# gau-nernst/pytorch-models

Hardware: AMD Instinct MI355X
Metric: ViT-B/16 images/s & Whisper-base audio-sec/s (BASELINE.json metric; value / unit / ms_per_step = the ViT-B/16 leg of configs[1], the Whisper-base leg of configs[2] is the "whisper" object) (higher is better)
Workload: dtype bf16; 1 GPU; ViT-B/16 bf16 forward, batch=256 per GPU, 224x224 (BASELINE configs[1]); per_gpu_batch=256, global_batch=256, parallelism=dp1, collective=none

## Files before the change

pytorch-models_amd/csrc/common.h:

```cpp
#pragma once
#include <hip/hip_runtime.h>
#include <stdint.h>

#include "../../include/pm_mi355x.h"

typedef __bf16 bf16;
typedef __attribute__((ext_vector_type(8))) __bf16 bf16x8;
typedef __attribute__((ext_vector_type(4))) __bf16 bf16x4;
typedef __attribute__((ext_vector_type(2))) __bf16 bf16x2;
typedef __attribute__((ext_vector_type(4))) float f32x4;
typedef __attribute__((ext_vector_type(2))) float f32x2;
typedef __attribute__((ext_vector_type(16))) float f32x16;
typedef __attribute__((ext_vector_type(4))) short s16x4;

#define PM_LDS __attribute__((address_space(3)))
#define PM_GLOBAL __attribute__((address_space(1)))

__device__ __forceinline__ float sum8_dpp(float v) {
  v += __builtin_bit_cast(float, __builtin_amdgcn_update_dpp(0, __builtin_bit_cast(int, v), 0xB1, 0xF, 0xF, true));
  v += __builtin_bit_cast(float, __builtin_amdgcn_update_dpp(0, __builtin_bit_cast(int, v), 0x4E, 0xF, 0xF, true));
  v += __builtin_bit_cast(float, __builtin_amdgcn_update_dpp(0, __builtin_bit_cast(int, v), 0x141, 0xF, 0xF, true));
  return v;
}

struct PmLnFold {
  const float* stats;
  const float* s;
  float* row_out;
};

#define PM_CHECK_LAUNCH()                                  \
  do {                                                     \
    if (hipGetLastError() != hipSuccess) return PM_ELAUNCH; \
  } while (0)

__device__ __forceinline__ float bf16_bits_to_f32(unsigned short b) { return __uint_as_float(((unsigned)b) << 16); }

#ifndef PM_GLDS_AUX
#define PM_GLDS_AUX 0
#endif
#ifndef PM_Y_NT
#define PM_Y_NT 1
#endif
template <typename V>
__device__ __forceinline__ void store_y(V* p, V v) {
#if PM_Y_NT
  __builtin_nontemporal_store(v, p);
#else
  *p = v;
#endif
}
__device__ __forceinline__ void glds16(const void* gsrc, void* lds_dst_wave_base) {
  __builtin_amdgcn_global_load_lds((const PM_GLOBAL void*)gsrc, (PM_LDS void*)lds_dst_wave_base, 16, 0, PM_GLDS_AUX);
}
#ifndef PM_GLDS_X_AUX
#define PM_GLDS_X_AUX 0
#endif
#ifndef PM_GLDS_W_AUX
#define PM_GLDS_W_AUX 0
#endif
template <int AUX>
__device__ __forceinline__ void glds16_aux(const void* gsrc, void* lds_dst_wave_base) {
  __builtin_amdgcn_global_load_lds((const PM_GLOBAL void*)gsrc, (PM_LDS void*)lds_dst_wave_base, 16, 0, AUX);
}

__device__ __forceinline__ void store_sc1_x4(f32x4* p, f32x4 v) {
  asm volatile("global_store_dwordx4 %0, %1, off sc1" ::"v"(p), "v"(v) : "memory");
}
__device__ __forceinline__ f32x4 load_sc1_x4(const f32x4* p) {
  f32x4 v;
  asm volatile("global_load_dwordx4 %0, %1, off sc1\n\ts_waitcnt vmcnt(0)" : "=v"(v) : "v"(p) : "memory");
  return v;
}

__device__ __forceinline__ f32x4 load_sc1_x4_async(const f32x4* p) {
  f32x4 v;
  asm volatile("global_load_dwordx4 %0, %1, off sc1" : "=v"(v) : "v"(p) : "memory");
  return v;
}
__device__ __forceinline__ void wait_loads(f32x4& a, f32x4& b, f32x4& c, f32x4& d) {
  asm volatile("s_waitcnt vmcnt(0)" : "+v"(a), "+v"(b), "+v"(c), "+v"(d)::"memory");
}

__device__ __forceinline__ void wait_vmcnt0() { asm volatile("s_waitcnt vmcnt(0)" ::: "memory"); }

__device__ __forceinline__ float erf_fast(float x) {
  const float ax = fabsf(x);
  const float t = __frcp_rn(fmaf(0.3275911f, ax, 1.0f));
  float p = fmaf(1.061405429f, t, -1.453152027f);
  p = fmaf(p, t, 1.421413741f);
  p = fmaf(p, t, -0.284496736f);
  p = fmaf(p, t, 0.254829592f);
  const float e = __expf(-ax * ax);
  const float r = fmaf(-p * t, e, 1.0f);
  return copysignf(r, x);
}

__device__ __forceinline__ float gelu_poly(float x) {
  const float xc = __builtin_amdgcn_fmed3f(x, -4.5f, 4.5f);
  const float t = fmaf(xc * xc, 2.0f / 20.25f, -1.0f);
  float q = 3.353692146e-03f;
  q = fmaf(q, t, -9.328538250e-03f);
  q = fmaf(q, t, 1.220852128e-02f);
  q = fmaf(q, t, -1.674404426e-02f);
  q = fmaf(q, t, 2.762940359e-02f);
  q = fmaf(q, t, -4.055576763e-02f);
  q = fmaf(q, t, 5.481856801e-02f);
  q = fmaf(q, t, -7.717196008e-02f);
  q = fmaf(q, t, 1.569021127e-01f);
  return x * fmaf(xc, q, 0.5f);
}

__device__ __forceinline__ f32x2 gelu_poly2(f32x2 x) {
  f32x2 xc;
  xc[0] = __builtin_amdgcn_fmed3f(x[0], -4.5f, 4.5f);
  xc[1] = __builtin_amdgcn_fmed3f(x[1], -4.5f, 4.5f);
  const f32x2 k1 = {2.0f / 20.25f, 2.0f / 20.25f}, m1 = {-1.0f, -1.0f}, half = {0.5f, 0.5f};
  const f32x2 t = __builtin_elementwise_fma(xc * xc, k1, m1);
  f32x2 q = {3.353692146e-03f, 3.353692146e-03f};
  q = __builtin_elementwise_fma(q, t, f32x2{-9.328538250e-03f, -9.328538250e-03f});
  q = __builtin_elementwise_fma(q, t, f32x2{1.220852128e-02f, 1.220852128e-02f});
  q = __builtin_elementwise_fma(q, t, f32x2{-1.674404426e-02f, -1.674404426e-02f});
  q = __builtin_elementwise_fma(q, t, f32x2{2.762940359e-02f, 2.762940359e-02f});
  q = __builtin_elementwise_fma(q, t, f32x2{-4.055576763e-02f, -4.055576763e-02f});
  q = __builtin_elementwise_fma(q, t, f32x2{5.481856801e-02f, 5.481856801e-02f});
  q = __builtin_elementwise_fma(q, t, f32x2{-7.717196008e-02f, -7.717196008e-02f});
  q = __builtin_elementwise_fma(q, t, f32x2{1.569021127e-01f, 1.569021127e-01f});
  return x * __builtin_elementwise_fma(xc, q, half);
// ... 53 lines not shown
```

pytorch-models_amd/csrc/linear_bf16.hip:

```cpp
#include <stdlib.h>

#include "common.h"
#ifndef PM_STATIC_PRIO
#define PM_STATIC_PRIO 1
#endif

int pm_linear_bf16_wide_launch(const void* x, int64_t ldx, int64_t x_rows_per_batch, int64_t x_batch_stride, const void* w,
                               int64_t ldw, const float* bias, const void* resid, int64_t ldr, int64_t resid_period, void* y,
                               int64_t ldy, int64_t M, int64_t N, int64_t K, int act, PmLnFold ln, hipStream_t st);
bool pm_linear_bf16_wide_applies(int64_t M, int64_t N, int64_t K, int act);
int pm_linear_bf16_tile_launch(int mi, const void* x, int64_t ldx, int64_t x_rows_per_batch, int64_t x_batch_stride,
                               const void* w, int64_t ldw, const float* bias, const void* resid, int64_t ldr,
                               int64_t resid_period, void* y, int64_t ldy, int64_t M, int64_t N, int64_t K, int act, PmLnFold ln,
                               hipStream_t st);
bool pm_linear_bf16_tile_applies(int64_t M, int64_t N, int64_t K, int act);
#ifdef PM_EXPERIMENTS
int pm_linear_bf16_sk_launch(const void* x, int64_t ldx, int64_t x_rows_per_batch, int64_t x_batch_stride, const void* w,
                             int64_t ldw, const float* bias, const void* resid, int64_t ldr, int64_t resid_period, void* y,
                             int64_t ldy, int64_t M, int64_t N, int64_t K, int act, PmLnFold ln, void* ws, hipStream_t st,
                             int mode);
bool pm_linear_bf16_hyb_applies(int64_t M, int64_t N, int64_t K, int act);
bool pm_linear_bf16_sk_applies(int64_t M, int64_t N, int64_t K, int act);
int64_t pm_linear_sk_ws_bytes();
#else
// ... 427 lines not shown
#undef PM_GO
  return PM_OK;
}

}

enum { PM_K_SMALL = 1, PM_K_PERSIST = 2, PM_K_WIDE = 3, PM_K_SK = 4, PM_K_HYB = 5, PM_K_TILE4 = 6, PM_K_TILE5 = 7 };
static int pm_linear_pick_kernel(int64_t M, int64_t N, int64_t K, bool persist_ok, bool wide_ok, bool sk_ok, bool hyb_ok,
                                 bool has_resid, bool tile_ok) {
  static const int forced = [] { const char* e = getenv("PM_GEMM_KERNEL"); return e ? atoi(e) : 0; }();
  static const bool use_sk = [] { const char* e = getenv("PM_GEMM_STREAMK"); return e && atoi(e) != 0; }();
  if (!use_sk && forced != PM_K_SK) sk_ok = false;
  static const bool use_hyb = [] { const char* e = getenv("PM_GEMM_HYBRID"); return e && atoi(e) != 0; }();
  if (!use_hyb && forced != PM_K_HYB) hyb_ok = false;
  if (forced == PM_K_SK && sk_ok) return PM_K_SK;
  if (forced == PM_K_HYB && hyb_ok) return PM_K_HYB;
  if (forced && forced != PM_K_SK) sk_ok = false;
  if (forced && forced != PM_K_HYB) hyb_ok = false;
  if (forced == PM_K_WIDE && wide_ok) return PM_K_WIDE;
  if ((forced == PM_K_TILE4 || forced == PM_K_TILE5) && tile_ok) return forced;
  static const bool use_tile = [] { const char* e = getenv("PM_GEMM_TILE"); return !e || atoi(e) != 0; }();
  if (!use_tile || forced) tile_ok = false;
  if (forced == PM_K_PERSIST && persist_ok) return PM_K_PERSIST;
  if (forced == PM_K_SMALL) return PM_K_SMALL;
  if (forced == PM_K_PERSIST) wide_ok = false;
  const double tm = (double)((M + 255) / 256), tw = tm * (double)((N + 255) / 256), tp = tm * (double)((N + 127) / 128);
  const double ts = (double)((M + 127) / 128) * (double)((N + 127) / 128);
  auto rounds = [](double t, double slots, double frac) {
    const double full = (double)(int64_t)(t / slots), rem = t - full * slots;
    return full + (rem > 0 ? frac + (1.0 - frac) * rem / slots : 0.0);
  };
  const double cs = rounds(ts, 512, 0.3) * 2.0 / (has_resid ? 0.65 : 0.7);
  const double cp = persist_ok ? rounds(tp, 256, 1.0) * 2.0 : 1e30;
  const double cw = wide_ok ? rounds(tw, 256, 1.0) * 4.0 / (has_resid ? 1.1 : 1.25) : 1e30;
  const double csk = sk_ok ? (tw / 256.0 + 0.25 * 768.0 / (double)K) * 4.0 / (has_resid ? 1.1 : 1.25) : 1e30;
  const double t5 = (double)((M + 319) / 320) * (double)((N + 255) / 256);
  const double ct4 = tile_ok ? rounds(tw, 256, 1.0) * 4.0 / (has_resid ? 1.1 : 1.25) : 1e30;
  const double ct5 = tile_ok ? rounds(t5, 256, 1.0) * 5.0 / (1.07 * (has_resid ? 1.1 : 1.25)) : 1e30;
  if (tile_ok) {
    const double bt = ct4 <= ct5 ? ct4 : ct5;
    if (bt <= cp && bt <= cs) return ct4 <= ct5 ? PM_K_TILE4 : PM_K_TILE5;
  }
  const double best = cw < cp ? (cw < cs ? cw : cs) : (cp < cs ? cp : cs);
  const double chyb = hyb_ok ? ((double)(int64_t)(tw / 256.0) + 0.5 + 0.25 * 768.0 / (double)K) * 4.0 / (has_resid ? 1.1 : 1.25) : 1e30;
  if (csk < 0.97 * best && csk <= chyb) return PM_K_SK;
  if (chyb < 0.97 * best) return PM_K_HYB;
  if (cw <= cp && cw <= cs) return PM_K_WIDE;
  return cp <= cs ? PM_K_PERSIST : PM_K_SMALL;
}

static int linear_impl(const void* x, int64_t ldx, int64_t x_rows_per_batch, int64_t x_batch_stride, const void* w,
                       int64_t ldw, const float* bias, const void* resid, int64_t ldr, int resid_dtype,
                       int64_t resid_period, void* y, int64_t ldy, int y_dtype, int64_t M, int64_t N, int64_t K, int act,
                       PmLnFold ln, void* stream, void* ws = nullptr, int64_t ws_bytes = 0) {
  if (!x || !w || !y || M < 0 || N <= 0 || K <= 0) return PM_EINVAL;
  const bool want_ln = ln.stats || ln.row_out;
  if ((ln.stats == nullptr) != (ln.s == nullptr)) return PM_EINVAL;
  if (ln.row_out && N % 64) return PM_EUNSUPPORTED;
  if (M == 0) return PM_OK;
  if (y_dtype != PM_BF16 && y_dtype != PM_F32) return PM_EINVAL;
  if (resid && resid_dtype != PM_BF16 && resid_dtype != PM_F32) return PM_EINVAL;
  if (K % 8 != 0) return PM_EUNSUPPORTED;
  if (ldx < 0 || ldw < K || ldy < N || (resid && ldr < N) || x_rows_per_batch < 0 || resid_period < 0) return PM_EINVAL;
  if (ldx % 8 || ldw % 8 || x_batch_stride % 8) return PM_EALIGN;
  if (((uintptr_t)x | (uintptr_t)w) & 15) return PM_EALIGN;
  const int vec_ok = (N % 4 == 0) && (ldy % 4 == 0) && (!resid || ldr % 4 == 0) &&
                     !((uintptr_t)y & (y_dtype == PM_F32 ? 15 : 7)) && !(bias && ((uintptr_t)bias & 15)) &&
                     !(resid && ((uintptr_t)resid & (resid_dtype == PM_F32 ? 15 : 7)));
  if (M > (1 << 30) || N > (1 << 30) || K > (1 << 30) || resid_period > (1 << 30)) return PM_EINVAL;
  hipStream_t st0 = (hipStream_t)stream;
  const bool out_vec16 = N % 8 == 0 && ldy % 8 == 0 && !((uintptr_t)y & 15);
  const bool wide_base = y_dtype == PM_BF16 && vec_ok && out_vec16 && !(resid && resid_dtype != PM_BF16) &&
                         !(resid && (ldr % 8 || ((uintptr_t)resid & 15))) &&
                         (x_rows_per_batch > 0 ? (M / x_rows_per_batch + 1) * x_batch_stride : M * ldx) < (1LL << 32) &&
                         N * ldw < (1LL << 32);
  bool wide_ok = wide_base && pm_linear_bf16_wide_applies(M, N, K, act) && !ln.row_out;
  const bool sk_ok = wide_base && ws && ws_bytes >= pm_linear_sk_ws_bytes() && !((uintptr_t)ws & 15) &&
                     pm_linear_bf16_sk_applies(M, N, K, act) && !(ln.row_out && act != PM_ACT_NONE);
  const bool persist_ok = (K % BK == 0) && (M >= 4096) && (y_dtype == PM_F32 || !vec_ok || out_vec16);
  const bool staged_ok = persist_ok && y_dtype == PM_BF16 && vec_ok && !(resid && resid_dtype == PM_F32);
  const bool hyb_ok = wide_base && ws && ws_bytes >= pm_linear_sk_ws_bytes() && !((uintptr_t)ws & 15) &&
                      pm_linear_bf16_hyb_applies(M, N, K, act) && !(ln.row_out && act != PM_ACT_NONE);
  const bool tile_ok = wide_base && pm_linear_bf16_tile_applies(M, N, K, act) && M % 8 == 0 && x_rows_per_batch == 0 &&
                       !(ln.stats && (resid || ln.row_out)) && !(ln.row_out && act != PM_ACT_NONE);
  int kernel;
  if (want_ln) {
    if (!staged_ok) return PM_EUNSUPPORTED;
    kernel = pm_linear_pick_kernel(M, N, K, true, wide_ok, sk_ok, hyb_ok, resid != nullptr, tile_ok);
    if (kernel == PM_K_SMALL) kernel = PM_K_PERSIST;
  } else {
    kernel = pm_linear_pick_kernel(M, N, K, persist_ok, wide_ok, sk_ok, hyb_ok, resid != nullptr, tile_ok);
  }
  if (kernel == PM_K_TILE4 || kernel == PM_K_TILE5) {
    const int rct = pm_linear_bf16_tile_launch(kernel == PM_K_TILE4 ? 4 : 5, x, ldx, x_rows_per_batch, x_batch_stride, w, ldw, bias,
                                               resid, ldr, resid_period, y, ldy, M, N, K, act, ln, st0);
    if (rct != PM_OK) return rct;
    PM_CHECK_LAUNCH();
    return PM_OK;
  }
  if (kernel == PM_K_SK || kernel == PM_K_HYB) {
    const int rck = pm_linear_bf16_sk_launch(x, ldx, x_rows_per_batch, x_batch_stride, w, ldw, bias, resid, ldr, resid_period, y,
                                             ldy, M, N, K, act, ln, ws, st0, kernel == PM_K_HYB ? 1 : 0);
    if (rck != PM_OK) return rck;
    PM_CHECK_LAUNCH();
    return PM_OK;
  }
  if (kernel == PM_K_WIDE) {
    const int rcw = pm_linear_bf16_wide_launch(x, ldx, x_rows_per_batch, x_batch_stride, w, ldw, bias, resid, ldr, resid_period, y,
                                               ldy, M, N, K, act, ln, st0);
    if (rcw != PM_OK) return rcw;
    PM_CHECK_LAUNCH();
    return PM_OK;
  }
  const bool big = kernel == PM_K_PERSIST;
  const int tiles_m = (int)((M + (big ? LBM : BM) - 1) / (big ? LBM : BM)), tiles_n = (int)((N + BN - 1) / BN);
  const int64_t nblk = (int64_t)tiles_m * tiles_n;
  if (nblk > 0x7fffffff) return PM_EINVAL;
  dim3 grid((unsigned)nblk);
  hipStream_t st = (hipStream_t)stream;
  int rc = (y_dtype == PM_F32)
               ? launch_act<true>(act, big, grid, st, (const bf16*)x, ldx, (const bf16*)w, ldw, bias, resid, ldr,
                                  resid_dtype == PM_F32, (int)resid_period, y, ldy, (int)M, (int)N, (int)K, tiles_n,
                                  (int)x_rows_per_batch, x_batch_stride, vec_ok, ln)
               : launch_act<false>(act, big, grid, st, (const bf16*)x, ldx, (const bf16*)w, ldw, bias, resid, ldr,
                                   resid_dtype == PM_F32, (int)resid_period, y, ldy, (int)M, (int)N, (int)K, tiles_n,
                                   (int)x_rows_per_batch, x_batch_stride, vec_ok, ln);
  if (rc != PM_OK) return rc;
  PM_CHECK_LAUNCH();
  return PM_OK;
}

extern "C" int pm_linear_bf16(const void* x, int64_t ldx, const void* w, int64_t ldw, const float* bias,
                              const void* resid, int64_t ldr, int resid_dtype, void* y, int64_t ldy, int y_dtype,
                              int64_t M, int64_t N, int64_t K, int act, void* stream) {
  if (ldx < K) return PM_EINVAL;
  return linear_impl(x, ldx, 0, 0, w, ldw, bias, resid, ldr, resid_dtype, 0, y, ldy, y_dtype, M, N, K, act, PmLnFold{}, stream);
}

extern "C" int pm_linear_bf16_ex(const void* x, int64_t ldx, int64_t x_rows_per_batch, int64_t x_batch_stride,
                                 const void* w, int64_t ldw, const float* bias, const void* resid, int64_t ldr,
                                 int resid_dtype, int64_t resid_period, void* y, int64_t ldy, int y_dtype, int64_t M,
                                 int64_t N, int64_t K, int act, void* stream) {
  return linear_impl(x, ldx, x_rows_per_batch, x_batch_stride, w, ldw, bias, resid, ldr, resid_dtype, resid_period, y, ldy,
                     y_dtype, M, N, K, act, PmLnFold{}, stream);
}

extern "C" int pm_linear_bf16_ln(const void* x, int64_t ldx, int64_t x_rows_per_batch, int64_t x_batch_stride,
                                 const void* w, int64_t ldw, const float* bias, const void* resid, int64_t ldr,
                                 int resid_dtype, int64_t resid_period, void* y, int64_t ldy, int y_dtype, int64_t M,
                                 int64_t N, int64_t K, int act, const float* ln_stats, const float* ln_s,
                                 float* ln_row_out, void* stream) {
  PmLnFold ln{ln_stats, ln_s, ln_row_out};
  return linear_impl(x, ldx, x_rows_per_batch, x_batch_stride, w, ldw, bias, resid, ldr, resid_dtype, resid_period, y, ldy,
                     y_dtype, M, N, K, act, ln, stream);
}

extern "C" int pm_linear_bf16_ws(const void* x, int64_t ldx, int64_t x_rows_per_batch, int64_t x_batch_stride,
                                 const void* w, int64_t ldw, const float* bias, const void* resid, int64_t ldr,
                                 int resid_dtype, int64_t resid_period, void* y, int64_t ldy, int y_dtype, int64_t M,
                                 int64_t N, int64_t K, int act, const float* ln_stats, const float* ln_s,
                                 float* ln_row_out, void* ws, int64_t ws_bytes, void* stream) {
  PmLnFold ln{ln_stats, ln_s, ln_row_out};
  return linear_impl(x, ldx, x_rows_per_batch, x_batch_stride, w, ldw, bias, resid, ldr, resid_dtype, resid_period, y, ldy,
                     y_dtype, M, N, K, act, ln, stream, ws, ws_bytes);
}

extern "C" int64_t pm_linear_ws_bytes(void) { return pm_linear_sk_ws_bytes(); }
// ... 55 lines not shown
```

pytorch-models_amd/csrc/linear_bf16_tile.hip:

```cpp
#include <cstdlib>

#include "common.h"

namespace {
#ifndef PM_TILE_RESID16
#define PM_TILE_RESID16 0
#endif
typedef unsigned u32x2 __attribute__((ext_vector_type(2)));
#ifndef PM_TILE_STAMPS
#define PM_TILE_STAMPS 0
#endif
#if PM_TILE_STAMPS
__device__ unsigned long long g_tile_stamps[256 * 16];
#define PM_TSTAMP(i_, cond_)                                                                       \
  do {                                                                                             \
    if ((cond_) && threadIdx.x == 0) g_tile_stamps[blockIdx.x * 16 + (i_)] = wall_clock64();        \
  } while (0)
#else
#define PM_TSTAMP(i_, cond_)
#endif

constexpr int TBN = 256, TBK = 64;
#ifndef PM_TGROUP_M
#define PM_TGROUP_M 4
#endif
constexpr int TGROUP_M = PM_TGROUP_M;

__device__ __forceinline__ bf16x8 tread(const char* tile, int row, int chunk) {
  return *(const bf16x8*)(tile + row * 128 + swz_pos(row, chunk) * 16);
}

__device__ __forceinline__ void ttile_coords(int t, int tiles_m, int tiles_n, int& tm, int& tn) {
  const int per = TGROUP_M * tiles_n;
  const int sr = t / per, r = t - sr * per;
  const int left = tiles_m - sr * TGROUP_M;
  const int gm = left < TGROUP_M ? left : TGROUP_M;
  tn = r / gm;
  tm = sr * TGROUP_M + (r - tn * gm);
}

enum { EPI_PLAIN = 0, EPI_LNC = 1, EPI_RES = 2 };

template <int MI, int ACT, int EPI>
__global__ __launch_bounds__(512, 2) void linear_bf16_tile_kernel(
    const bf16* __restrict__ X, int64_t ldx, const bf16* __restrict__ W, int64_t ldw, const float* __restrict__ bias,
    const bf16* resid, int64_t ldr, int resid_period, bf16* Y, int64_t ldy, int M, int N, int K, int tiles_m, int tiles_n,
    int x_rows_per_batch, int64_t x_batch_stride, PmLnFold ln) {
  constexpr bool LNC = EPI == EPI_LNC, RES = EPI == EPI_RES;
  constexpr int RPF = MI > 4 ? 1 : 2;
  constexpr int BM = 64 * MI, WR = 16 * MI;
  constexpr int STAGE = (BM + TBN) * 128;
  constexpr int XP = MI, WP = 4;
  __shared__ __attribute__((aligned(16))) char smem[2 * STAGE + 8 * 2048];
  const int tid = threadIdx.x, lane = tid & 63;
  const int wave = __builtin_amdgcn_readfirstlane(tid >> 6);
  const int wm = wave >> 1, wn = wave & 1;
  const int ntiles = tiles_m * tiles_n;

  const int xcd = blockIdx.x & 7, local = blockIdx.x >> 3, nloc = gridDim.x >> 3;
  const int cq = ntiles >> 3, cr = ntiles & 7;
  const int tbase = xcd * cq + (xcd < cr ? xcd : cr), tcount = cq + (xcd < cr ? 1 : 0);
  const int my_tiles = local < tcount ? (tcount - local + nloc - 1) / nloc : 0;
  const int nk = K / TBK;
  const int P = my_tiles * nk;

  const char* xbase[XP];
  const char* wbase[WP];
  const uint32_t lsw = (uint32_t)(((lane & 7) ^ (lane >> 4)) * 16);
  const uint32_t xl0 = (uint32_t)(lane >> 3) * (uint32_t)(ldx * 2), wl0 = (uint32_t)(lane >> 3) * (uint32_t)(ldw * 2);
  int pp = 0, pp_kt = 0, pp_tile = 0, pp_buf = 0;
#define PM_TSTAGE_NEXT()                                                                                             \
  if (pp < P) {                                                                                                      \
    if (pp_kt == 0) {                                                                                                \
      int tm_, tn_;                                                                                                  \
      ttile_coords(tbase + local + pp_tile * nloc, tiles_m, tiles_n, tm_, tn_);                                      \
      _Pragma("unroll") for (int i = 0; i < XP; ++i) {                                                               \
        int r_ = tm_ * BM + wave * (8 * MI) + i * 8;                                                                 \
        r_ = r_ < M - 8 ? r_ : M - 8;                                                                                \
        xbase[i] = (const char*)X + (int64_t)r_ * ldx * 2;                                                           \
      }                                                                                                              \
      _Pragma("unroll") for (int i = 0; i < WP; ++i) {                                                               \
        int r_ = tn_ * TBN + wave * 32 + i * 8;                                                                      \
        r_ = r_ < N - 8 ? r_ : N - 8;                                                                                \
        wbase[i] = (const char*)W + (int64_t)r_ * ldw * 2;                                                           \
      }                                                                                                              \
    }                                                                                                                \
    char* xs_ = smem + pp_buf * STAGE;                                                                               \
    const uint32_t kb_ = (uint32_t)(pp_kt * (TBK * 2));                                                              \
                                                               \
    _Pragma("unroll") for (int i = 0; i < XP; ++i) {                                                                 \
      uint32_t ph_ = (uint32_t)(((wave * MI + i) & 1) * 64);                                                         \
      asm volatile("" : "+s"(ph_));                                                                                  \
      glds16_aux<PM_GLDS_X_AUX>(xbase[i] + (uint32_t)(xl0 + kb_ + (lsw ^ ph_)), xs_ + (wave * (8 * MI) + i * 8) * 128); \
    }                                                                                                                \
    _Pragma("unroll") for (int i = 0; i < WP; ++i) {                                                                 \
      uint32_t ph_ = (uint32_t)((i & 1) * 64);                                                                       \
      asm volatile("" : "+s"(ph_));                                                                                  \
      glds16_aux<PM_GLDS_W_AUX>(wbase[i] + (uint32_t)(wl0 + kb_ + (lsw ^ ph_)), xs_ + BM * 128 + (wave * 32 + i * 8) * 128); \
    }                                                                                                                \
    ++pp;                                                                                                            \
    pp_buf ^= 1;                                                                                                     \
    if (++pp_kt == nk) { pp_kt = 0; ++pp_tile; }                                                                     \
  }

  f32x4 acc[8][MI];
#pragma unroll
  for (int j = 0; j < 8; ++j)
#pragma unroll
    for (int i = 0; i < MI; ++i) acc[j][i] = f32x4{0.f, 0.f, 0.f, 0.f};

  if (wave >= 4) __builtin_amdgcn_s_setprio(1);
  PM_TSTAGE_NEXT();
  const int fr = lane & 15, fq = lane >> 4;
  int buf = 0, kt = 0, ti = 0;
  f32x2 lnst[MI];
#pragma unroll
  for (int i = 0; i < MI; ++i) lnst[i] = f32x2{0.f, 1.f};
  bf16x4 rv[RES ? RPF + 1 : 1][4];

#ifdef PM_TILE_ABLATE_RESID
#define PM_TILE_RESID_LOAD(dst_, ptr_) { asm volatile("" ::"v"(ptr_)); dst_ = bf16x4{}; }
#else
#define PM_TILE_RESID_LOAD(dst_, ptr_) dst_ = *(const bf16x4*)(ptr_)
#endif
#define PM_TLOAD_RESID(q_, slot_, m0_, n0_, fr_, fq_)                                                                \
  {                                                                                                                  \
    const int hf_ = (q_) / MI, i_ = (q_) - hf_ * MI;                                                                 \
    int r0_ = (m0_) + i_ * 16;                                                                                       \
    int mm_ = r0_ + (fr_);                                                                                           \
    mm_ = mm_ < M ? mm_ : M - 1;                                                                                     \
    r0_ = r0_ < M - 16 ? r0_ : M - 16;        \
    const char* rb_;                                                                                                 \
    uint32_t ro_;                                                                                                    \
    if (resid_period) {                                                                                              \
      rb_ = (const char*)resid;                                                                                      \
      ro_ = (uint32_t)(mm_ % resid_period) * (uint32_t)(ldr * 2);                                                    \
// ... 65 lines not shown
#pragma unroll
    for (int ss = 0; ss < 2; ++ss) {
      bf16x8 a[8], b[MI];
#ifndef PM_TILE_ASM_READS
#define PM_TILE_ASM_READS 1
#endif
#if PM_TILE_ASM_READS
#define PM_TREAD1(dst_, base_, off_) asm volatile("ds_read_b128 %0, %1 offset:%2" : "=v"(dst_) : "v"(base_), "n"(off_))
#define PM_TWAIT(n_, j_)                                                                                             \
  if constexpr (MI == 5)                                                                                             \
    asm volatile("s_waitcnt lgkmcnt(%6)" : "+v"(a[j_]), "+v"(b[0]), "+v"(b[1]), "+v"(b[2]), "+v"(b[3]), "+v"(b[MI - 1]) : "n"(n_)); \
  else                                                                                                               \
    asm volatile("s_waitcnt lgkmcnt(%5)" : "+v"(a[j_]), "+v"(b[0]), "+v"(b[1]), "+v"(b[2]), "+v"(b[3]) : "n"(n_));
#define PM_TREADS()                                                                                                  \
  {                                                                                                                  \
    const uint32_t sw_ = (uint32_t)(((ss * 4 + fq) ^ ((fr >> 1) & 7)) * 16 + fr * 128);                              \
    const uint32_t xb_ = (uint32_t)(uintptr_t)(PM_LDS const char*)xcur + (uint32_t)(wm * WR * 128) + sw_;            \
    const uint32_t wb_ = (uint32_t)(uintptr_t)(PM_LDS const char*)xcur + (uint32_t)(wn * 128 * 128) + sw_;           \
    _Pragma("unroll") for (int i = 0; i < MI; ++i) PM_TREAD1(b[i], xb_, i * 2048);                                   \
    _Pragma("unroll") for (int j = 0; j < 8; ++j) PM_TREAD1(a[j], wb_, BM * 128 + j * 2048);                         \
  }
#else
#define PM_TWAIT(n_, j_)
#define PM_TREADS()                                                                                                  \
  {                                                                                                                  \
    _Pragma("unroll") for (int i = 0; i < MI; ++i) b[i] = tread(xcur, wm * WR + i * 16 + fr, ss * 4 + fq);           \
    a[0] = tread(wcur, wn * 128 + fr, ss * 4 + fq);                                                                  \
    __builtin_amdgcn_sched_barrier(0);                                                                               \
    _Pragma("unroll") for (int j = 1; j < 8; ++j) {                                                                  \
      a[j] = tread(wcur, wn * 128 + j * 16 + fr, ss * 4 + fq);                                                       \
      __builtin_amdgcn_sched_barrier(0);                                                                             \
    }                                                                                                                \
  }
#endif
#define PM_TWAIT_J(j_)                                                                                               \
  {                                                                                                                  \
    if ((j_) == 0) { PM_TWAIT(7, 0) } else if ((j_) == 1) { PM_TWAIT(6, 1) } else if ((j_) == 2) { PM_TWAIT(5, 2) }  \
    else if ((j_) == 3) { PM_TWAIT(4, 3) } else if ((j_) == 4) { PM_TWAIT(3, 4) } else if ((j_) == 5) { PM_TWAIT(2, 5) } \
    else if ((j_) == 6) { PM_TWAIT(1, 6) } else { PM_TWAIT(0, 7) }                                                   \
  }
      if (kt == 0 && ss == 0) {
        PM_TREADS();
        const f32x4 zero = {0.f, 0.f, 0.f, 0.f};
#pragma unroll
        for (int j = 0; j < 8; ++j) {
          PM_TWAIT_J(j);
#pragma unroll
          for (int i = 0; i < MI; ++i) acc[j][i] = __builtin_amdgcn_mfma_f32_16x16x32_bf16(a[j], b[i], zero, 0, 0, 0);
          __builtin_amdgcn_sched_barrier(0);
        }
      } else {
        PM_TREADS();
#pragma unroll
        for (int j = 0; j < 8; ++j) {
          PM_TWAIT_J(j);
#pragma unroll
          for (int i = 0; i < MI; ++i) acc[j][i] = __builtin_amdgcn_mfma_f32_16x16x32_bf16(a[j], b[i], acc[j][i], 0, 0, 0);
          __builtin_amdgcn_sched_barrier(0);
        }
      }
#undef PM_TREADS
#undef PM_TWAIT_J
#undef PM_TWAIT
      if (MI > 4) __builtin_amdgcn_sched_barrier(0);
      if (PM_TILE_ISSUE_SPLIT && ss == 0 && wave >= 4) {
        PM_TSTAGE_NEXT();
        __builtin_amdgcn_sched_barrier(0);
      }
    }
    buf ^= 1;
    if (++kt < nk) continue;

    kt = 0;
#ifdef PM_TILE_ABLATE_EPI
    {
#pragma unroll
      for (int j = 0; j < 8; ++j)
#pragma unroll
        for (int i = 0; i < MI; ++i) asm volatile("" ::"v"(acc[j][i]));
      ++ti;
      continue;
    }
#endif
    int tm, tn;
    ttile_coords(tbase + local + ti * nloc, tiles_m, tiles_n, tm, tn);
    ++ti;
    const int m0 = tm * BM + wm * WR, n0 = tn * TBN + wn * 128;
    PM_TSTAMP(1, ti == 1);
    char* stg = smem + 2 * STAGE + wave * 2048;
    int el = lane;
    asm volatile("" : "+v"(el));
    const int srow = el >> 3, sch = el & 7, efr = el & 15, efq = el >> 4;
    const uint32_t ylane = (uint32_t)srow * (uint32_t)(ldy * 2) + (uint32_t)sch * 16;
    const int mleft = M - m0 - srow;
    char* const wr_ptr = stg + efr * 128 + (efq & 1) * 8;
    const int wr_sw = (efr >> 1) & 7;
    const char* const rd_ptr0 = stg + srow * 128 + ((sch ^ ((srow >> 1) & 7)) * 16);
    const char* const rd_ptr1 = stg + (srow + 8) * 128 + ((sch ^ (((srow + 8) >> 1) & 7)) * 16);
    if constexpr (RES && MI > 4) {
#pragma unroll
      for (int q = 0; q < RPF; ++q) PM_TLOAD_RESID(q, q, m0, n0, efr, efq);
    }
    f32x4 bvec[4], svec[LNC ? 4 : 1], bnxt[4], snxt[LNC ? 4 : 1];
#define PM_TLOAD_BIAS(bd_, sd_, hf_)                                                                                  \
  _Pragma("unroll") for (int jj = 0; jj < 4; ++jj) {                                                                   \
    int n = n0 + (hf_) * 64 + jj * 16 + efq * 4;                                                                       \
    n = n < N ? n : N - 4;                                                     \
    bd_[jj] = bias ? *(const f32x4*)((const char*)bias + (uint32_t)n * 4) : f32x4{0.f, 0.f, 0.f, 0.f};                 \
    if constexpr (LNC) sd_[jj] = *(const f32x4*)((const char*)ln.s + (uint32_t)n * 4);                                 \
  }
    PM_TLOAD_BIAS(bvec, svec, 0);
#pragma unroll
    for (int hf = 0; hf < 2; ++hf) {
      if (hf == 1) {
#pragma unroll
        for (int jj = 0; jj < 4; ++jj) {
          bvec[jj] = bnxt[jj];
          if constexpr (LNC) svec[jj] = snxt[jj];
        }
      }
#pragma unroll
      for (int i = 0; i < MI; ++i) {
        if (hf == 0 && i == MI - 1) PM_TLOAD_BIAS(bnxt, snxt, 1);
        const int q = hf * MI + i;
        if constexpr (RES) {
          if (q + RPF < 2 * MI) PM_TLOAD_RESID(q + RPF, (q + RPF) % (RPF + 1), m0, n0, efr, efq);
          PM_TRESID_UNSWAP(q % (RPF + 1))
        }
        bf16x4 o[4];
#pragma unroll
        for (int jj = 0; jj < 4; ++jj) {
          f32x4 v;
          if constexpr (LNC) {
            const float mu = lnst[i][0], rstd = lnst[i][1];
#pragma unroll
            for (int r = 0; r < 4; ++r) v[r] = fmaf(rstd, acc[hf * 4 + jj][i][r] - mu * svec[jj][r], bvec[jj][r]);
          } else {
            v = acc[hf * 4 + jj][i] + bvec[jj];
          }
          v = apply_act4<ACT>(v);
          if constexpr (RES) {
#pragma unroll
            for (int r = 0; r < 4; ++r) v[r] += (float)rv[q % (RPF + 1)][jj][r];
          }
#pragma unroll
          for (int r = 0; r < 4; ++r) o[jj][r] = (bf16)v[r];
          *(bf16x4*)(wr_ptr + (((jj * 2 + (efq >> 1)) ^ wr_sw) * 16)) = o[jj];
        }
        if (!LNC && ln.row_out) {
          bf16x8 ones;
#pragma unroll
          for (int e = 0; e < 8; ++e) ones[e] = (bf16)1.0f;
          const bf16x8 f0 = __builtin_shufflevector(o[0], o[1], 0, 1, 2, 3, 4, 5, 6, 7);
          const bf16x8 f1 = __builtin_shufflevector(o[2], o[3], 0, 1, 2, 3, 4, 5, 6, 7);
          const f32x4 zero = {0.f, 0.f, 0.f, 0.f};
          f32x4 d1 = __builtin_amdgcn_mfma_f32_16x16x32_bf16(ones, f0, zero, 0, 0, 0);
          d1 = __builtin_amdgcn_mfma_f32_16x16x32_bf16(ones, f1, d1, 0, 0, 0);
          f32x4 d2 = __builtin_amdgcn_mfma_f32_16x16x32_bf16(f0, f0, zero, 0, 0, 0);
          d2 = __builtin_amdgcn_mfma_f32_16x16x32_bf16(f1, f1, d2, 0, 0, 0);
          const int rr = efr & 3;
          const float s2 = rr == 0 ? d2[0] : rr == 1 ? d2[1] : rr == 2 ? d2[2] : d2[3];
          const int np = N >> 6;
          char* const sb = (char*)ln.row_out + ((int64_t)(m0 + i * 16) * np + ((n0 + hf * 64) >> 6)) * 8;
          if (efq == (efr >> 2) && m0 + i * 16 + efr < M && n0 + hf * 64 < N)
            *(f32x2*)(sb + (uint32_t)efr * (uint32_t)(np * 8)) = f32x2{d1[0], s2};
        }
#pragma unroll
        for (int p = 0; p < 2; ++p) {
          const bf16x8 ov = *(const bf16x8*)(p ? rd_ptr1 : rd_ptr0);
          char* const yb = (char*)Y + ((int64_t)(m0 + i * 16 + p * 8) * ldy + n0 + hf * 64) * 2;
#ifdef PM_TILE_ABLATE_STORE
          asm volatile("" ::"v"(ov), "v"(yb + ylane));
#else
          if (i * 16 + p * 8 < mleft && n0 + hf * 64 + sch * 8 < N)
            store_y((bf16x8*)(yb + ylane), ov);
#endif
        }
        PM_TSTAMP(2 + q, ti == 1);
      }
    }
#ifndef PM_TILE_NO_ACC_KILL
#pragma unroll
    for (int j = 0; j < 8; ++j)
#pragma unroll
      for (int i = 0; i < MI; ++i) asm volatile("" : "=v"(acc[j][i]));
#endif
  }
#undef PM_TSTAGE_NEXT
#undef PM_TLOAD_RESID
#undef PM_TLOAD_BIAS
}

}

#if PM_TILE_STAMPS
extern "C" int pm_debug_tile_stamps(void* out) {
  return hipMemcpyFromSymbol(out, HIP_SYMBOL(g_tile_stamps), sizeof(unsigned long long) * 256 * 16) == hipSuccess ? 0 : 1;
}
#endif

int pm_linear_bf16_tile_launch(int mi, const void* x, int64_t ldx, int64_t x_rows_per_batch, int64_t x_batch_stride,
                               const void* w, int64_t ldw, const float* bias, const void* resid, int64_t ldr,
                               int64_t resid_period, void* y, int64_t ldy, int64_t M, int64_t N, int64_t K, int act, PmLnFold ln,
                               hipStream_t st) {
  const int bm = 64 * mi;
  const int tiles_m = (int)((M + bm - 1) / bm), tiles_n = (int)((N + TBN - 1) / TBN);
  if (ln.stats && (resid || ln.row_out)) return PM_EUNSUPPORTED;
  const int epi = ln.stats ? EPI_LNC : resid ? EPI_RES : EPI_PLAIN;
#define PM_TGO(MI_, A, L)                                                                                              \
  hipLaunchKernelGGL((linear_bf16_tile_kernel<MI_, A, L>), dim3(256), dim3(512), 0, st, (const bf16*)x, ldx, (const bf16*)w, \
                     ldw, bias, (const bf16*)resid, ldr, (int)resid_period, (bf16*)y, ldy, (int)M, (int)N, (int)K, tiles_m, \
                     tiles_n, (int)x_rows_per_batch, x_batch_stride, ln)
#define PM_TGO_MI(MI_)                                             \
  if (act == PM_ACT_NONE) {                                        \
    if (epi == EPI_LNC) PM_TGO(MI_, PM_ACT_NONE, EPI_LNC);         \
    else if (epi == EPI_RES) PM_TGO(MI_, PM_ACT_NONE, EPI_RES);    \
    else PM_TGO(MI_, PM_ACT_NONE, EPI_PLAIN);                      \
  } else if (act == PM_ACT_GELU) {                                 \
    if (epi == EPI_LNC) PM_TGO(MI_, PM_ACT_GELU, EPI_LNC);         \
    else if (epi == EPI_RES) PM_TGO(MI_, PM_ACT_GELU, EPI_RES);    \
    else PM_TGO(MI_, PM_ACT_GELU, EPI_PLAIN);                      \
  } else {                                                         \
    return PM_EUNSUPPORTED;                                        \
  }
  if (mi == 4) { PM_TGO_MI(4) }
  else if (mi == 5) { PM_TGO_MI(5) }
  else return PM_EINVAL;
#undef PM_TGO_MI
#undef PM_TGO
  return PM_OK;
}

bool pm_linear_bf16_tile_applies(int64_t M, int64_t N, int64_t K, int act) {
  if (act != PM_ACT_NONE && act != PM_ACT_GELU) return false;
  if (K % TBK || N % 8) return false;
  return M >= 4096;
}
```

Before: 29790 images/s.

## Rewrite tile GEMM epilogue with register permlane transpose and scalar addressing

Replaces the LDS-staged epilogue of the tiled bf16 GEMM with a register-only path that uses permlane16_swap to form 16-byte output vectors, dropping the per-wave 2KB staging buffer from shared memory. It also moves tile base pointers into scalar registers with uniform strides for output, residual, bias and LN partial-sum addressing. A bounds-free FULL specialization is used for interior tiles. The dispatcher now requires ldy and ldr below 2^24 because 32-bit offsets are used. Risks are a different global store pattern (16 rows by 2 chunks instead of 8-row groups) and more code paths.

```diff
diff --git a/pytorch-models_amd/csrc/common.h b/pytorch-models_amd/csrc/common.h
--- a/pytorch-models_amd/csrc/common.h
+++ b/pytorch-models_amd/csrc/common.h
@@ -44,6 +44,14 @@
 #endif
 template <typename V>
 __device__ __forceinline__ void store_y(V* p, V v) {
+#if PM_Y_NT
+  __builtin_nontemporal_store(v, p);
+#else
+  *p = v;
+#endif
+}
+template <typename V>
+__device__ __forceinline__ void store_y(PM_GLOBAL V* p, V v) {
 #if PM_Y_NT
   __builtin_nontemporal_store(v, p);
 #else
diff --git a/pytorch-models_amd/csrc/linear_bf16.hip b/pytorch-models_amd/csrc/linear_bf16.hip
--- a/pytorch-models_amd/csrc/linear_bf16.hip
+++ b/pytorch-models_amd/csrc/linear_bf16.hip
@@ -533,7 +533,8 @@
   const bool hyb_ok = wide_base && ws && ws_bytes >= pm_linear_sk_ws_bytes() && !((uintptr_t)ws & 15) &&
                       pm_linear_bf16_hyb_applies(M, N, K, act) && !(ln.row_out && act != PM_ACT_NONE);
   const bool tile_ok = wide_base && pm_linear_bf16_tile_applies(M, N, K, act) && M % 8 == 0 && x_rows_per_batch == 0 &&
-                       !(ln.stats && (resid || ln.row_out)) && !(ln.row_out && act != PM_ACT_NONE);
+                       !(ln.stats && (resid || ln.row_out)) && !(ln.row_out && act != PM_ACT_NONE) && ldy < (1 << 24) &&
+                       !(resid && ldr >= (1 << 24));
   int kernel;
   if (want_ln) {
     if (!staged_ok) return PM_EUNSUPPORTED;
diff --git a/pytorch-models_amd/csrc/linear_bf16_tile.hip b/pytorch-models_amd/csrc/linear_bf16_tile.hip
--- a/pytorch-models_amd/csrc/linear_bf16_tile.hip
+++ b/pytorch-models_amd/csrc/linear_bf16_tile.hip
@@ -6,7 +6,21 @@
 #ifndef PM_TILE_RESID16
 #define PM_TILE_RESID16 0
 #endif
+#ifndef PM_TILE_EPI_REGS
+#define PM_TILE_EPI_REGS 1
+#endif
+#ifndef PM_TILE_EPI_ADDR
+#define PM_TILE_EPI_ADDR 1
+#endif
+#ifndef PM_TILE_EPI_FAST
+#define PM_TILE_EPI_FAST 1
+#endif
 typedef unsigned u32x2 __attribute__((ext_vector_type(2)));
+typedef unsigned u32x4 __attribute__((ext_vector_type(4)));
+template <bool B>
+struct TBool {
+  static constexpr bool value = B;
+};
 #ifndef PM_TILE_STAMPS
 #define PM_TILE_STAMPS 0
 #endif
@@ -51,7 +65,7 @@
   constexpr int BM = 64 * MI, WR = 16 * MI;
   constexpr int STAGE = (BM + TBN) * 128;
   constexpr int XP = MI, WP = 4;
-  __shared__ __attribute__((aligned(16))) char smem[2 * STAGE + 8 * 2048];
+  __shared__ __attribute__((aligned(16))) char smem[2 * STAGE + (PM_TILE_EPI_REGS ? 0 : 8 * 2048)];
   const int tid = threadIdx.x, lane = tid & 63;
   const int wave = __builtin_amdgcn_readfirstlane(tid >> 6);
   const int wm = wave >> 1, wn = wave & 1;
@@ -283,6 +297,7 @@
       continue;
     }
 #endif
+#if !PM_TILE_EPI_REGS && !PM_TILE_EPI_ADDR && !PM_TILE_EPI_FAST
     int tm, tn;
     ttile_coords(tbase + local + ti * nloc, tiles_m, tiles_n, tm, tn);
     ++ti;
@@ -380,6 +395,269 @@
         PM_TSTAMP(2 + q, ti == 1);
       }
     }
+#undef PM_TLOAD_BIAS
+#else
+    int tm, tn;
+    ttile_coords(tbase + local + ti * nloc, tiles_m, tiles_n, tm, tn);
+    ++ti;
+    const int m0 = tm * BM + wm * WR, n0 = tn * TBN + wn * 128;
+    PM_TSTAMP(1, ti == 1);
+    int el = lane;
+    asm volatile("" : "+v"(el));
+    const int efr = el & 15, efq = el >> 4;
+    auto epilogue = [&](auto full_c) __attribute__((always_inline)) {
+      constexpr bool FULL = decltype(full_c)::value;
+#if PM_TILE_EPI_REGS == 0
+      char* stg = smem + 2 * STAGE + wave * 2048;
+      const int srow = el >> 3, sch = el & 7;
+      const int yrl = srow, yfl = sch * 8;
+      constexpr int YROFF = 8, YFOFF = 0;
+      char* const wr_ptr = stg + efr * 128 + (efq & 1) * 8;
+      const int wr_sw = (efr >> 1) & 7;
+      const char* const rd_ptr0 = stg + srow * 128 + ((sch ^ ((srow >> 1) & 7)) * 16);
+      const char* const rd_ptr1 = stg + (srow + 8) * 128 + ((sch ^ (((srow + 8) >> 1) & 7)) * 16);
+#elif PM_TILE_EPI_REGS == 1
+      const int yrl = efr, yfl = (efq & 1) * 16 + (efq & ~1) * 4;
+      constexpr int YROFF = 0, YFOFF = 32;
+#else
+      const int yrl = efr & 7, yfl = ((efr >> 3) * 2 + (efq & 1)) * 16 + (efq & ~1) * 4;
+      constexpr int YROFF = 8, YFOFF = 0;
+#endif
+      const uint32_t ldy2 = (uint32_t)(ldy * 2);
+      const uint32_t ylane = (uint32_t)yrl * ldy2 + (uint32_t)yfl * 2;
+      const int mleft = M - m0 - yrl;
+      const int nleft = N - n0 - yfl;
+      [[maybe_unused]] PM_GLOBAL char* ytile = (PM_GLOBAL char*)Y + ((int64_t)m0 * ldy + n0) * 2;
+      [[maybe_unused]] uint32_t ystep = 16 * ldy2;
+      [[maybe_unused]] PM_GLOBAL char* yrow = ytile;
+      const int np = N >> 6;
+      [[maybe_unused]] PM_GLOBAL char* stile = (PM_GLOBAL char*)ln.row_out + ((int64_t)m0 * np + (n0 >> 6)) * 8;
+      [[maybe_unused]] uint32_t sstep = 16 * (uint32_t)(np * 8);
+      [[maybe_unused]] PM_GLOBAL char* spart = stile;
+      const uint32_t ldr2 = (uint32_t)(ldr * 2);
+      const int rt0 = FULL ? m0 : (m0 < M - WR ? m0 : M - WR);
+      [[maybe_unused]] const PM_GLOBAL char* rtile = (const PM_GLOBAL char*)resid + ((int64_t)rt0 * ldr + (FULL ? n0 : 0)) * 2;
+      [[maybe_unused]] uint32_t rstep = FULL ? 16 * ldr2 : 0u;
+      [[maybe_unused]] const uint32_t rlane =
+          (uint32_t)efr * ldr2 + (uint32_t)(PM_TILE_RESID16 ? ((efq & 1) * 16 + (efq & ~1) * 4) * 2 : efq * 8);
+      [[maybe_unused]] const int rrl = efr + m0 - rt0, rrlim = M - 1 - rt0;
+      [[maybe_unused]] const PM_GLOBAL char* btile = (const PM_GLOBAL char*)bias + (uint32_t)n0 * 4;
+      [[maybe_unused]] const PM_GLOBAL char* ctile = (const PM_GLOBAL char*)ln.s + (uint32_t)n0 * 4;
+#if PM_TILE_EPI_ADDR
+      asm volatile("" : "+s"(ytile), "+s"(ystep), "+s"(stile), "+s"(sstep));
+      if constexpr (RES) asm volatile("" : "+s"(rtile), "+s"(rstep));
+      yrow = ytile;
+      spart = stile;
+#endif
+      [[maybe_unused]] const PM_GLOBAL char* rrow = rtile + (uint64_t)rstep * (MI <= 4 ? RPF - 1 : 0);
+#define PM_TLOAD_RESID_CH(q_, slot_)                                                                                 \
+  {                                                                                                                  \
+    const int hf_ = (q_) / MI, i_ = (q_) - hf_ * MI;                                                          \
+    const PM_GLOBAL char* rb_;                                                                                       \
+    uint32_t ro_;                                                                                                    \
+    if (resid_period) {                                                                                              \
+      int mm_ = m0 + i_ * 16 + efr;                                                                                  \
+      if (!FULL) mm_ = mm_ < M ? mm_ : M - 1;                                                                        \
+      rb_ = (const PM_GLOBAL char*)resid + (FULL ? (uint32_t)n0 * 2 : 0u);                                              \
+      ro_ = (uint32_t)(mm_ % resid_period) * ldr2;                                                                   \
+      if (FULL) ro_ += rlane - (uint32_t)efr * ldr2;                                                                 \
+    } else {                                                                                                         \
+      if (i_ == 0) rrow = rtile; else rrow += rstep;                                                                 \
+      asm volatile("" : "+s"(rrow));                                                                                 \
+      rb_ = rrow;                                                                                                    \
+      if (FULL) {                                                                                                    \
+        ro_ = rlane;                                                                                                 \
+        asm volatile("" : "+v"(ro_));                \
+      }                                                                                                              \
+      else {                                                                                                         \
+        int rr_ = rrl + i_ * 16;                                                                                     \
+        rr_ = rr_ < rrlim ? rr_ : rrlim;                                                                             \
+        ro_ = (uint32_t)rr_ * ldr2;                                                                                  \
+      }                                                                                                              \
+    }                                                                                                                \
+    if (PM_TILE_RESID16) {                                                                                           \
+      _Pragma("unroll") for (int k_ = 0; k_ < 2; ++k_) {                                                             \
+        bf16x8 l_;                                                                                                   \
+        if (FULL) l_ = *(const PM_GLOBAL bf16x8*)(rb_ + ro_ + (hf_ * 128 + k_ * 64));                                          \
+        else {                                                                                                       \
+          int nn_ = n0 + hf_ * 64 + (2 * k_ + (efq & 1)) * 16 + (efq & ~1) * 4;                                      \
+          nn_ = nn_ < N - 8 ? nn_ : N - 8;                                   \
+          l_ = *(const PM_GLOBAL bf16x8*)(rb_ + (uint32_t)(ro_ + (uint32_t)nn_ * 2));                                \
+        }                                                                                                            \
+        rv[slot_][2 * k_] = __builtin_shufflevector(l_, l_, 0, 1, 2, 3);                                             \
+        rv[slot_][2 * k_ + 1] = __builtin_shufflevector(l_, l_, 4, 5, 6, 7);                                         \
+      }                                                                                                              \
+    } else {                                                                                                         \
+      _Pragma("unroll") for (int jj = 0; jj < 4; ++jj) {                                                             \
+        if (FULL) PM_TILE_RESID_LOAD(rv[slot_][jj], rb_ + ro_ + (hf_ * 128 + jj * 32));                              \
+        else {                                                                                                       \
+          int nn_ = n0 + hf_ * 64 + jj * 16 + efq * 4;                                                               \
+          nn_ = nn_ < N ? nn_ : N - 4;                                       \
+          PM_TILE_RESID_LOAD(rv[slot_][jj], rb_ + (uint32_t)(ro_ + (uint32_t)nn_ * 2));                              \
+        }                                                                                                            \
+      }                                                                                                              \
+    }                                                                                                                \
+  }
+#if PM_TILE_EPI_ADDR
+#define PM_TLOAD_RESID_E(q_, slot_) PM_TLOAD_RESID_CH(q_, slot_)
+#else
+#define PM_TLOAD_RESID_E(q_, slot_) PM_TLOAD_RESID(q_, slot_, m0, n0, efr, efq)
+#endif
+      if constexpr (RES && MI > 4) {
+#pragma unroll
+        for (int q = 0; q < RPF; ++q) PM_TLOAD_RESID_E(q, q);
+      }
+      f32x4 bvec[4], svec[LNC ? 4 : 1], bnxt[4], snxt[LNC ? 4 : 1];
+#define PM_TLOAD_BIAS(bd_, sd_, hf_)                                                                                  \
+  _Pragma("unroll") for (int jj = 0; jj < 4; ++jj) {                                                                   \
+    if (PM_TILE_EPI_ADDR && FULL) {                                                                                    \
+      bd_[jj] = f32x4{0.f, 0.f, 0.f, 0.f};                                                                             \
+      if (bias) {                                                                                                      \
+        uint32_t o_ = (uint32_t)efq * 16;                                                                              \
+        asm volatile("" : "+v"(o_));                   \
+        bd_[jj] = *(const PM_GLOBAL f32x4*)(btile + o_ + ((hf_) * 256 + jj * 64));                                     \
+      }                                                                                                                \
+      if constexpr (LNC) {                                                                                             \
+        uint32_t o_ = (uint32_t)efq * 16;                                                                              \
+        asm volatile("" : "+v"(o_));                                                                                   \
+        sd_[jj] = *(const PM_GLOBAL f32x4*)(ctile + o_ + ((hf_) * 256 + jj * 64));                                     \
+      }                                                                                                                \
+    } else {                                                                                                           \
+      int n = n0 + (hf_) * 64 + jj * 16 + efq * 4;                                                                     \
+      if (!FULL) n = n < N ? n : N - 4;                                        \
+      bd_[jj] = bias ? *(const f32x4*)((const char*)bias + (uint32_t)n * 4) : f32x4{0.f, 0.f, 0.f, 0.f};               \
+      if constexpr (LNC) sd_[jj] = *(const f32x4*)((const char*)ln.s + (uint32_t)n * 4);                               \
+    }                                                                                                                  \
+  }
+      PM_TLOAD_BIAS(bvec, svec, 0);
+#pragma unroll
+      for (int hf = 0; hf < 2; ++hf) {
+        if (hf == 1) {
+#pragma unroll
+          for (int jj = 0; jj < 4; ++jj) {
+            bvec[jj] = bnxt[jj];
+            if constexpr (LNC) svec[jj] = snxt[jj];
+          }
+        }
+#pragma unroll
+        for (int i = 0; i < MI; ++i) {
+          if (hf == 0 && i == MI - 1) PM_TLOAD_BIAS(bnxt, snxt, 1);
+          const int q = hf * MI + i;
+          if constexpr (RES) {
+            if (q + RPF < 2 * MI) PM_TLOAD_RESID_E(q + RPF, (q + RPF) % (RPF + 1));
+            PM_TRESID_UNSWAP(q % (RPF + 1))
+          }
+          [[maybe_unused]] float mu = lnst[i][0], rstd = lnst[i][1];
+          if (LNC && FULL) asm volatile("" : "+v"(mu), "+v"(rstd));
+          bf16x4 o[4];
+#pragma unroll
+          for (int jj = 0; jj < 4; ++jj) {
+            f32x4 v;
+            if constexpr (LNC) {
+#pragma unroll
+              for (int r = 0; r < 4; ++r) v[r] = fmaf(rstd, acc[hf * 4 + jj][i][r] - mu * svec[jj][r], bvec[jj][r]);
+            } else {
+              v = acc[hf * 4 + jj][i] + bvec[jj];
+            }
+            v = apply_act4<ACT>(v);
+            if constexpr (RES) {
+#pragma unroll
+              for (int r = 0; r < 4; ++r) v[r] += (float)rv[q % (RPF + 1)][jj][r];
+            }
+#pragma unroll
+            for (int r = 0; r < 4; ++r) o[jj][r] = (bf16)v[r];
+#if PM_TILE_EPI_REGS == 0
+            *(bf16x4*)(wr_ptr + (((jj * 2 + (efq >> 1)) ^ wr_sw) * 16)) = o[jj];
+#endif
+          }
+          if (!LNC && ln.row_out) {
+            bf16x8 ones;
+#pragma unroll
+            for (int e = 0; e < 8; ++e) ones[e] = (bf16)1.0f;
+            const bf16x8 f0 = __builtin_shufflevector(o[0], o[1], 0, 1, 2, 3, 4, 5, 6, 7);
+            const bf16x8 f1 = __builtin_shufflevector(o[2], o[3], 0, 1, 2, 3, 4, 5, 6, 7);
+            const f32x4 zero = {0.f, 0.f, 0.f, 0.f};
+            f32x4 d1 = __builtin_amdgcn_mfma_f32_16x16x32_bf16(ones, f0, zero, 0, 0, 0);
+            d1 = __builtin_amdgcn_mfma_f32_16x16x32_bf16(ones, f1, d1, 0, 0, 0);
+            f32x4 d2 = __builtin_amdgcn_mfma_f32_16x16x32_bf16(f0, f0, zero, 0, 0, 0);
+            d2 = __builtin_amdgcn_mfma_f32_16x16x32_bf16(f1, f1, d2, 0, 0, 0);
+            const int rr = efr & 3;
+            const float s2 = rr == 0 ? d2[0] : rr == 1 ? d2[1] : rr == 2 ? d2[2] : d2[3];
+#if PM_TILE_EPI_ADDR
+            PM_GLOBAL char* const sb = spart + hf * 8;
+#else
+            PM_GLOBAL char* const sb = (PM_GLOBAL char*)ln.row_out + ((int64_t)(m0 + i * 16) * np + ((n0 + hf * 64) >> 6)) * 8;
+#endif
+            if (efq == (efr >> 2) && (FULL || (m0 + i * 16 + efr < M && n0 + hf * 64 < N)))
+              *(PM_GLOBAL f32x2*)(sb + (uint32_t)efr * (uint32_t)(np * 8)) = f32x2{d1[0], s2};
+          }
+          uint32_t yl = ylane;
+          if (PM_TILE_EPI_ADDR && FULL) asm volatile("" : "+v"(yl));
+          bf16x8 ov[2];
+#if PM_TILE_EPI_REGS == 0
+          ov[0] = *(const bf16x8*)rd_ptr0;
+          ov[1] = *(const bf16x8*)rd_ptr1;
+#else
+          u32x4 sv[2];
+#pragma unroll
+          for (int k = 0; k < 2; ++k) {
+            u32x2 p_ = __builtin_bit_cast(u32x2, o[2 * k]), q_ = __builtin_bit_cast(u32x2, o[2 * k + 1]);
+#pragma unroll
+            for (int w = 0; w < 2; ++w) {
+              const auto r_ = __builtin_amdgcn_permlane16_swap(p_[w], q_[w], false, false);
+              p_[w] = r_[0];
+              q_[w] = r_[1];
+            }
+            sv[k] = u32x4{p_[0], p_[1], q_[0], q_[1]};
+          }
+#if PM_TILE_EPI_REGS == 2
+          {
+            u32x4 t0, t1;
+#pragma unroll
+            for (int w = 0; w < 4; ++w) {
+              t0[w] = (unsigned)__builtin_amdgcn_update_dpp((int)sv[0][w], (int)sv[1][w], 0x128, 0xF, 0xC, false);
+              t1[w] = (unsigned)__builtin_amdgcn_update_dpp((int)sv[1][w], (int)sv[0][w], 0x128, 0xF, 0x3, false);
+            }
+            sv[0] = t0;
+            sv[1] = t1;
+          }
+#endif
+          ov[0] = __builtin_bit_cast(bf16x8, sv[0]);
+          ov[1] = __builtin_bit_cast(bf16x8, sv[1]);
+#endif
+#pragma unroll
+          for (int s = 0; s < 2; ++s) {
+#if PM_TILE_EPI_ADDR
+            PM_GLOBAL char* yb = yrow;
+            if (YROFF && s) {
+              yb += 8 * ldy2;
+              asm volatile("" : "+s"(yb));
+            }
+            yb += (hf * 64 + YFOFF * s) * 2;
+#else
+            PM_GLOBAL char* const yb = (PM_GLOBAL char*)Y + ((int64_t)(m0 + i * 16 + YROFF * s) * ldy + n0 + hf * 64 + YFOFF * s) * 2;
+#endif
+#ifdef PM_TILE_ABLATE_STORE
+            asm volatile("" ::"v"(ov[s]), "v"(yb + yl));
+#else
+            if (FULL || (i * 16 + YROFF * s < mleft && hf * 64 + YFOFF * s < nleft)) store_y((PM_GLOBAL bf16x8*)(yb + yl), ov[s]);
+#endif
+          }
+#if PM_TILE_EPI_ADDR
+          if (i == MI - 1) { yrow = ytile; spart = stile; } else { yrow += ystep; spart += sstep; }
+          asm volatile("" : "+s"(yrow), "+s"(spart));
+#endif
+          PM_TSTAMP(2 + q, ti == 1);
+        }
+      }
+#undef PM_TLOAD_RESID_E
+#undef PM_TLOAD_RESID_CH
+#undef PM_TLOAD_BIAS
+    };
+    constexpr bool FAST = PM_TILE_EPI_FAST > 1 || (PM_TILE_EPI_FAST == 1 && !(LNC && MI > 4));
+    if (FAST && m0 + WR <= M && n0 + 128 <= N) epilogue(TBool<true>{});
+    else epilogue(TBool<false>{});
+#endif
 #ifndef PM_TILE_NO_ACC_KILL
 #pragma unroll
     for (int j = 0; j < 8; ++j)
@@ -389,7 +667,6 @@
   }
 #undef PM_TSTAGE_NEXT
 #undef PM_TLOAD_RESID
-#undef PM_TLOAD_BIAS
 }
 
 }
```

Measured after the change: 28710 images/s. 3.6% lower.
